# ErlerPhilipp/points2surf

Hardware: NVIDIA H100
Metric: SDF queries/sec at grid_res=256 (higher is better)
Workload: dtype f16 operands / f32 accumulate (wgmma); hi/lo split f16 (fp32-level) for FC tails and guard-band recompute

## Files before the change

### points2surf_b200/csrc/net_tc.cu

```cuda
#include "model.cuh"
#include "tc_ptx.cuh"

namespace p2s {

using namespace ptx;

namespace {

constexpr int kTile = 64;
constexpr int kWG = 2;
constexpr int kThreads = 128 * kWG;
constexpr uint32_t kAct2Bytes = kTile * 128 * 2;
template <bool PRECISE>
struct Cfg {
    static constexpr int kChunks = PRECISE ? 1 : 4;
    static constexpr int kSplit = 8 / kChunks;
    static constexpr uint32_t kChunkBytes = PRECISE ? 65536u : 32768u;
    static constexpr uint32_t kW3Bytes = kChunks * kChunkBytes;
    static constexpr uint32_t kMidScale = PRECISE ? 2u : 1u;
    static constexpr uint32_t kMidBytes = (8192u + 8192u + 16384u) * kMidScale;
    static constexpr uint32_t kPerqBytes = PRECISE ? 16384u : 8192u;
    static constexpr uint32_t kOffMid = kW3Bytes;
    static constexpr uint32_t kWgPerq = kAct2Bytes * kMidScale;
    static constexpr uint32_t kWgWq = kWgPerq + kPerqBytes;
    static constexpr uint32_t kWgBytes = kWgWq + 192 * 4;
    static constexpr uint32_t kOffWg = kOffMid + kMidBytes;
    static constexpr uint32_t kOffBias = kOffWg + kWG * kWgBytes;
    static constexpr uint32_t kSmemBytes = kOffBias + 320 * 4;
};
static_assert(Cfg<false>::kSmemBytes <= 232448 && Cfg<true>::kSmemBytes <= 232448, "shared memory budget");

struct Seg {
    const float* ptr;
    int n;
    int tiles;
    int center;
};

struct PassParams {
    Seg seg[2];
    const float* query;
    const float* R;
    int tiles_per_query;
    int B;
    const float* W0;
    const float* b0;
    int num_mid;
    int mid_N[3];
    const uint8_t* mid_img[3];
    const float* mid_bias[3];
    int perq_layer;
    const uint8_t* perq_img;
    const uint8_t* w3_img;
    float* out;
};

__device__ __forceinline__ uint32_t pack_relu(float a, float b) {
    uint32_t r;
    asm("cvt.rn.relu.satfinite.f16x2.f32 %0, %1, %2;" : "=r"(r) : "f"(b), "f"(a));
    return r;
}
__device__ __forceinline__ void pack_relu_split(float a, float b, uint32_t& hi, uint32_t& lo) {
    hi = pack_relu(a, b);
    const float2 hf = __half22float2(*reinterpret_cast<const __half2*>(&hi));
    lo = pack_half2(fmaxf(a, 0.f) - hf.x, fmaxf(b, 0.f) - hf.y);
}
template <bool PRECISE>
__device__ __forceinline__ void pack_act(float a, float b, uint32_t& hi, uint32_t& lo) {
    if (PRECISE) pack_relu_split(a, b, hi, lo);
    else hi = pack_relu(a, b);
}

template <bool PRECISE, int R>
__device__ __forceinline__ void mid_mma(float (&d)[R], const uint32_t (&a)[4], const uint32_t (&al)[4], uint64_t w, uint64_t w_lo, uint32_t acc) {
    if (R == 32) {
        auto& d32 = reinterpret_cast<float (&)[32]>(d);
        if (PRECISE) { wgmma_rs_n64(d32, al, w, acc); wgmma_rs_n64(d32, a, w_lo, 1); wgmma_rs_n64(d32, a, w, 1); }
        else wgmma_rs_n64(d32, a, w, acc);
    } else {
        auto& d64 = reinterpret_cast<float (&)[64]>(d);
        if (PRECISE) { wgmma_rs_n128(d64, al, w, acc); wgmma_rs_n128(d64, a, w_lo, 1); wgmma_rs_n128(d64, a, w, 1); }
        else wgmma_rs_n128(d64, a, w, acc);
    }
}

template <bool PRECISE>
__global__ void __launch_bounds__(kThreads, 1) pointnet_pass_kernel(const PassParams p) {
    using C = Cfg<PRECISE>;
    constexpr int kL = PRECISE ? 4 : 1;
    extern __shared__ __align__(1024) uint8_t smem[];
    float* s_bias = reinterpret_cast<float*>(smem + C::kOffBias);
    const int tid = threadIdx.x, wg = tid >> 7, t = tid & 127, lane = tid & 31, q4 = lane & 3;
    const int r0 = (t >> 5) * 16 + (lane >> 2);
    const int part = blockIdx.x % C::kSplit;
    const int stream = blockIdx.x / C::kSplit, nstreams = gridDim.x / C::kSplit;
    const int nq = (p.B > stream) ? (p.B - stream + nstreams - 1) / nstreams : 0;
    const int tpq = p.tiles_per_query;
    uint32_t mid_off[3] = {0, 0, 0};
    {
        uint32_t o = 0;
        for (int l = 0; l < p.num_mid; ++l) { mid_off[l] = o; o += (uint32_t)p.mid_N[l] * 128u * C::kMidScale; }
    }

    if (nq > 0) {
        const uint4* src = reinterpret_cast<const uint4*>(p.w3_img + (size_t)part * C::kW3Bytes);
        uint4* dst = reinterpret_cast<uint4*>(smem);
        for (uint32_t i = tid; i < C::kW3Bytes / 16; i += kThreads) dst[i] = src[i];
        for (int l = 0; l < p.num_mid; ++l) {
            if (l == p.perq_layer) continue;
            const uint4* s = reinterpret_cast<const uint4*>(p.mid_img[l]);
            uint4* d = reinterpret_cast<uint4*>(smem + C::kOffMid + mid_off[l]);
            for (uint32_t i = tid; i < (uint32_t)p.mid_N[l] * 8u * C::kMidScale; i += kThreads) d[i] = s[i];
        }
    }
    {
        int off = 0;
        for (int l = 0; l < p.num_mid; ++l) {
            for (int i = tid; i < p.mid_N[l]; i += kThreads) s_bias[off + i] = p.mid_bias[l][i];
            off += p.mid_N[l];
        }
        for (int i = tid; i < 64; i += kThreads) s_bias[256 + i] = p.b0[i];
    }
    fence_proxy_async_smem();
    __syncthreads();

    uint8_t* wsm = smem + C::kOffWg + wg * C::kWgBytes;
    uint8_t* act2 = wsm;
    uint8_t* perq = wsm + C::kWgPerq;
    float* wq = reinterpret_cast<float*>(wsm + C::kWgWq);
    const float* s_b0 = s_bias + 256;
    const uint32_t bar_id = 1 + (uint32_t)wg;
    auto wg_sync = [&]() { asm volatile("bar.sync %0, 128;" ::"r"(bar_id) : "memory"); };
    const uint64_t dsc_act2 = make_smem_desc(smem_u32(act2), 128, 2048);
    const uint64_t dsc_w3 = make_smem_desc(smem_u32(smem), 128, 2048);
    uint64_t dsc_mid[3], dsc_mid_lo[3];
    for (int l = 0; l < 3; ++l) {
        const bool pq = l == p.perq_layer;
        dsc_mid[l] = make_smem_desc(pq ? smem_u32(perq) : smem_u32(smem + C::kOffMid) + mid_off[l], 128, 1024);
        dsc_mid_lo[l] = dsc_mid[l] + (uint64_t)((pq ? 8192u : (uint32_t)p.mid_N[l] * 128u) >> 4);
    }

    for (int qi = wg; qi < nq; qi += kWG) {
        const size_t q = (size_t)stream + (size_t)qi * nstreams;
        wg_sync();
        if (t < 64) {
            const float w0 = p.W0[t * 3 + 0], w1 = p.W0[t * 3 + 1], w2 = p.W0[t * 3 + 2];
            float r[9] = {1.f, 0.f, 0.f, 0.f, 1.f, 0.f, 0.f, 0.f, 1.f};
            if (p.R) {
#pragma unroll
                for (int i = 0; i < 9; ++i) r[i] = p.R[q * 9 + i];
            }
            wq[0 * 64 + t] = w0 * r[0] + w1 * r[3] + w2 * r[6];
            wq[1 * 64 + t] = w0 * r[1] + w1 * r[4] + w2 * r[7];
            wq[2 * 64 + t] = w0 * r[2] + w1 * r[5] + w2 * r[8];
        }
        if (p.perq_layer >= 0) {
            const uint4* s = reinterpret_cast<const uint4*>(p.perq_img + q * C::kPerqBytes);
            uint4* d = reinterpret_cast<uint4*>(perq);
            for (uint32_t i = t; i < C::kPerqBytes / 16; i += 128) d[i] = s[i];
            fence_proxy_async_smem();
        }
        wg_sync();
        float rmax[4 * C::kChunks];
#pragma unroll
        for (int i = 0; i < 4 * C::kChunks; ++i) rmax[i] = -INFINITY;
        for (int tq = 0; tq < tpq; ++tq) {
            const int sgi = tq < p.seg[0].tiles ? 0 : 1;
            const Seg& sg = p.seg[sgi];
            float cx = 0.f, cy = 0.f, cz = 0.f;
            if (sg.center) { cx = p.query[q * 3 + 0]; cy = p.query[q * 3 + 1]; cz = p.query[q * 3 + 2]; }
            float px[2], py[2], pz[2];
#pragma unroll
            for (int h = 0; h < 2; ++h) {
                int local = (tq - (sgi ? p.seg[0].tiles : 0)) * kTile + r0 + 8 * h;
                if (local >= sg.n) local = 0;
                const float* src = sg.ptr + (q * sg.n + local) * 3;
                px[h] = src[0] - cx; py[h] = src[1] - cy; pz[h] = src[2] - cz;
            }
            uint32_t a[4][4], al[4][kL];
#pragma unroll
            for (int kk = 0; kk < 4; ++kk) {
#pragma unroll
                for (int hc = 0; hc < 2; ++hc) {
                    const int ch = kk * 16 + hc * 8 + 2 * q4;
                    const float2 wx = *reinterpret_cast<const float2*>(wq + 0 * 64 + ch);
                    const float2 wy = *reinterpret_cast<const float2*>(wq + 1 * 64 + ch);
                    const float2 wz = *reinterpret_cast<const float2*>(wq + 2 * 64 + ch);
                    const float2 bb = *reinterpret_cast<const float2*>(s_b0 + ch);
#pragma unroll
                    for (int h = 0; h < 2; ++h) {
                        const float v0 = fmaf(wx.x, px[h], fmaf(wy.x, py[h], fmaf(wz.x, pz[h], bb.x)));
                        const float v1 = fmaf(wx.y, px[h], fmaf(wy.y, py[h], fmaf(wz.y, pz[h], bb.y)));
                        pack_act<PRECISE>(v0, v1, a[kk][hc * 2 + h], al[kk][PRECISE ? hc * 2 + h : 0]);
                    }
                }
            }
            int boff = 0;
            for (int l = 0; l < p.num_mid; ++l) {
                const float* bl = s_bias + boff;
                const uint64_t w = dsc_mid[l], w_lo = dsc_mid_lo[l];
                if (l < p.num_mid - 1) {
                    float d[32];
#pragma unroll
                    for (int i = 0; i < 32; ++i) d[i] = 0.f;
                    wgmma_fence();
#pragma unroll
                    for (int ks = 0; ks < 4; ++ks)
                        mid_mma<PRECISE>(d, a[ks], reinterpret_cast<const uint32_t (&)[4]>(al[PRECISE ? ks : 0]), w + (uint64_t)(ks * 16), w_lo + (uint64_t)(ks * 16), ks > 0);
                    wgmma_commit();
                    wgmma_wait<0>();
                    fence_regs(d);
#pragma unroll
                    for (int j = 0; j < 8; ++j) {
                        const float2 bb = *reinterpret_cast<const float2*>(bl + 8 * j + 2 * q4);
                        pack_act<PRECISE>(d[4 * j] + bb.x, d[4 * j + 1] + bb.y, a[j >> 1][(j & 1) * 2], al[j >> 1][PRECISE ? (j & 1) * 2 : 0]);
                        pack_act<PRECISE>(d[4 * j + 2] + bb.x, d[4 * j + 3] + bb.y, a[j >> 1][(j & 1) * 2 + 1], al[j >> 1][PRECISE ? (j & 1) * 2 + 1 : 0]);
                    }
                } else {
                    float d[64];
#pragma unroll
                    for (int i = 0; i < 64; ++i) d[i] = 0.f;
                    wgmma_fence();
#pragma unroll
                    for (int ks = 0; ks < 4; ++ks)
                        mid_mma<PRECISE>(d, a[ks], reinterpret_cast<const uint32_t (&)[4]>(al[PRECISE ? ks : 0]), w + (uint64_t)(ks * 16), w_lo + (uint64_t)(ks * 16), ks > 0);
                    wgmma_commit();
                    wgmma_wait<0>();
                    fence_regs(d);
                    wg_sync();
#pragma unroll
                    for (int j = 0; j < 16; ++j) {
                        const int k = 8 * j + 2 * q4;
                        const float2 bb = *reinterpret_cast<const float2*>(bl + k);
#pragma unroll
                        for (int h = 0; h < 2; ++h) {
                            const int pt = r0 + 8 * h;
                            const uint32_t off = (uint32_t)(pt >> 3) * 2048u + (uint32_t)j * 128u + (uint32_t)(pt & 7) * 16u + (uint32_t)q4 * 4u;
                            uint32_t hi, lo = 0;
                            pack_act<PRECISE>(d[4 * j + 2 * h] + bb.x, d[4 * j + 2 * h + 1] + bb.y, hi, lo);
                            *reinterpret_cast<uint32_t*>(act2 + off) = hi;
                            if (PRECISE) *reinterpret_cast<uint32_t*>(act2 + kAct2Bytes + off) = lo;
                        }
                    }
                    fence_proxy_async_smem();
                    wg_sync();
                }
                boff += p.mid_N[l];
            }
#pragma unroll
            for (int c = 0; c < C::kChunks; ++c) {
                float d0[32], d1[32];
#pragma unroll
                for (int i = 0; i < 32; ++i) { d0[i] = 0.f; d1[i] = 0.f; }
                const uint64_t wa = dsc_w3 + (uint64_t)((uint32_t)c * (C::kChunkBytes >> 4)), wb = wa + (uint64_t)(16384u >> 4);
                wgmma_fence();
#pragma unroll
                for (int ks = 0; ks < 8; ++ks) {
                    const uint64_t x = dsc_act2 + (uint64_t)(ks * 16), o = (uint64_t)(ks * 16);
                    if (PRECISE) {
                        const uint64_t x_lo = x + (uint64_t)(kAct2Bytes >> 4), lo = (uint64_t)(32768u >> 4);
                        wgmma_ss_n64(d0, wa + lo + o, x, ks > 0); wgmma_ss_n64(d0, wa + o, x_lo, 1); wgmma_ss_n64(d0, wa + o, x, 1);
                        wgmma_ss_n64(d1, wb + lo + o, x, ks > 0); wgmma_ss_n64(d1, wb + o, x_lo, 1); wgmma_ss_n64(d1, wb + o, x, 1);
                    } else {
                        wgmma_ss_n64(d0, wa + o, x, ks > 0);
                        wgmma_ss_n64(d1, wb + o, x, ks > 0);
                    }
                }
                wgmma_commit();
                wgmma_wait<0>();
                fence_regs(d0);
                fence_regs(d1);
#pragma unroll
                for (int j = 0; j < 8; ++j) {
                    rmax[4 * c + 0] = fmaxf(rmax[4 * c + 0], fmaxf(d0[4 * j], d0[4 * j + 1]));
                    rmax[4 * c + 1] = fmaxf(rmax[4 * c + 1], fmaxf(d0[4 * j + 2], d0[4 * j + 3]));
                    rmax[4 * c + 2] = fmaxf(rmax[4 * c + 2], fmaxf(d1[4 * j], d1[4 * j + 1]));
                    rmax[4 * c + 3] = fmaxf(rmax[4 * c + 3], fmaxf(d1[4 * j + 2], d1[4 * j + 3]));
                }
            }
        }
#pragma unroll
        for (int i = 0; i < 4 * C::kChunks; ++i) {
            rmax[i] = fmaxf(rmax[i], __shfl_xor_sync(0xffffffffu, rmax[i], 1));
            rmax[i] = fmaxf(rmax[i], __shfl_xor_sync(0xffffffffu, rmax[i], 2));
        }
        if (q4 == 0) {
#pragma unroll
            for (int i = 0; i < 4 * C::kChunks; ++i)
                p.out[q * 1024 + (size_t)((part * C::kChunks + (i >> 2)) * 128 + ((i >> 1) & 1) * 64 + r0 + (i & 1) * 8)] = rmax[i];
        }
    }
}

__global__ void pack_kmajor_kernel(const float* __restrict__ W, int rows, int K, int row0, uint32_t sbo, uint8_t* __restrict__ img, int lo) {
    int e = blockIdx.x * blockDim.x + threadIdx.x;
    if (e >= rows * K) return;
    int r = e / K, k = e % K;
    uint32_t off = (uint32_t)(r >> 3) * sbo + (uint32_t)(k >> 3) * 128u + (uint32_t)(r & 7) * 16u + (uint32_t)(k & 7) * 2u;
    const float w = W[(size_t)(row0 + r) * K + k];
    const __half h = __float2half_rn(w);
    *reinterpret_cast<__half*>(img + off) = lo ? __float2half_rn(w - __half2float(h)) : h;
}

__global__ void pack_perq_kernel(const float* __restrict__ W, int64_t B, uint8_t* __restrict__ img) {
    int64_t e = (int64_t)blockIdx.x * blockDim.x + threadIdx.x;
    if (e >= B * 4096) return;
    int64_t b = e >> 12;
    int r = (int)((e >> 6) & 63), k = (int)(e & 63);
    uint32_t off = (uint32_t)(r >> 3) * 1024u + (uint32_t)(k >> 3) * 128u + (uint32_t)(r & 7) * 16u + (uint32_t)(k & 7) * 2u;
    *reinterpret_cast<__half*>(img + b * 8192 + off) = __float2half_rn(W[e]);
}

__global__ void __launch_bounds__(256) fold_w1_kernel(const float* __restrict__ W1, const float* __restrict__ T, int64_t B, uint8_t* __restrict__ img) {
    __shared__ float sW[64][65];
    __shared__ __align__(16) float sT[64][68];
    const int64_t b = blockIdx.x;
    const int tid = threadIdx.x;
    for (int e = tid; e < 4096; e += 256) {
        const int r = e >> 6, c = e & 63;
        sW[r][c] = W1[e];
        sT[r][c] = T[b * 4096 + e] + (r == c ? 1.0f : 0.0f);
    }
    __syncthreads();
    const int o = tid >> 2, i0 = (tid & 3) * 16;
    float acc[16];
#pragma unroll
    for (int i = 0; i < 16; ++i) acc[i] = 0.f;
    for (int j = 0; j < 64; ++j) {
        const float w = sW[o][j];
#pragma unroll
        for (int i4 = 0; i4 < 4; ++i4) {
            const float4 t4 = *reinterpret_cast<const float4*>(&sT[j][i0 + 4 * i4]);
            acc[4 * i4 + 0] = fmaf(w, t4.x, acc[4 * i4 + 0]);
            acc[4 * i4 + 1] = fmaf(w, t4.y, acc[4 * i4 + 1]);
            acc[4 * i4 + 2] = fmaf(w, t4.z, acc[4 * i4 + 2]);
            acc[4 * i4 + 3] = fmaf(w, t4.w, acc[4 * i4 + 3]);
        }
    }
    uint8_t* dst = img + b * 8192 + (uint32_t)(o >> 3) * 1024u + (uint32_t)(o & 7) * 16u;
#pragma unroll
    for (int h = 0; h < 2; ++h) {
        uint32_t v[4];
#pragma unroll
        for (int e = 0; e < 4; ++e) v[e] = pack_half2(acc[h * 8 + 2 * e], acc[h * 8 + 2 * e + 1]);
        *reinterpret_cast<uint4*>(dst + (uint32_t)(i0 / 8 + h) * 128u) = make_uint4(v[0], v[1], v[2], v[3]);
    }
}

__global__ void fold_fc3_kernel(const float* __restrict__ W1, const float* __restrict__ Wfc3, const float* __restrict__ bfc3,
                                float* __restrict__ G, float* __restrict__ g0) {
    const int oi = blockIdx.x;
    const int o = oi >> 6, i = oi & 63;
    const int k = threadIdx.x;
    float acc = 0.f;
    for (int j = 0; j < 64; ++j) acc = fmaf(W1[o * 64 + j], Wfc3[(size_t)(j * 64 + i) * 256 + k], acc);
    G[(size_t)oi * 256 + k] = acc;
    if (k == 0) {
        float b = W1[o * 64 + i];
        for (int j = 0; j < 64; ++j) b = fmaf(W1[o * 64 + j], bfc3[j * 64 + i], b);
        g0[oi] = b;
    }
}

__global__ void transpose64_kernel(const float* __restrict__ in, float* __restrict__ out, int64_t B) {
    int64_t e = (int64_t)blockIdx.x * blockDim.x + threadIdx.x;
    if (e >= B * 4096) return;
    int64_t b = e >> 12;
    int i = (int)((e >> 6) & 63), j = (int)(e & 63);
    out[e] = in[b * 4096 + j * 64 + i];
}

__global__ void guard_flag_kernel(const float* __restrict__ logits, int od, int64_t B, float band, int32_t* __restrict__ list, int* __restrict__ count, int64_t base, int64_t cap) {
    int64_t i = (int64_t)blockIdx.x * blockDim.x + threadIdx.x;
    if (i >= B) return;
    if (fabsf(logits[i * od + od - 1]) < band) {
        int slot = atomicAdd(count, 1);
        if (slot < cap) list[slot] = (int32_t)(base + i);
    }
}
__global__ void guard_gather_kernel(const float* __restrict__ src, const int32_t* __restrict__ list, int n, int row_floats, float* __restrict__ dst) {
    int64_t e = (int64_t)blockIdx.x * blockDim.x + threadIdx.x;
    if (e >= (int64_t)n * row_floats) return;
    int i = (int)(e / row_floats), j = (int)(e % row_floats);
    dst[e] = src[(int64_t)list[i] * row_floats + j];
}
__global__ void guard_scatter_kernel(const float* __restrict__ src, const int32_t* __restrict__ list, int n, int od, float* __restrict__ logits) {
    int i = blockIdx.x * blockDim.x + threadIdx.x;
    if (i >= n) return;
    for (int j = 0; j < od; ++j) logits[(int64_t)list[i] * od + j] = src[i * od + j];
}
__global__ void guard_scatter_rows_kernel(const float* __restrict__ src, const int32_t* __restrict__ list, int n, int row_floats, float* __restrict__ dst) {
    int64_t e = (int64_t)blockIdx.x * blockDim.x + threadIdx.x;
    if (e >= (int64_t)n * row_floats) return;
    int i = (int)(e / row_floats), j = (int)(e % row_floats);
    dst[(int64_t)list[i] * row_floats + j] = src[e];
}

}

struct TcStack {
    uint8_t* w3_img = nullptr;
    uint8_t* mid_img[3] = {nullptr, nullptr, nullptr};
    uint8_t* w3_img_p = nullptr;
    uint8_t* mid_img_p[3] = {nullptr, nullptr, nullptr};
    const float* mid_bias[3] = {nullptr, nullptr, nullptr};
    int mid_N[3] = {0, 0, 0};
    int num_mid = 0;
    const float* W0 = nullptr;
    const float* b0 = nullptr;
    const float* b3 = nullptr;
};

struct TcFc {
    const Layer* L = nullptr;
    const uint8_t* img = nullptr;
};
struct TcStnFc { TcFc fc1, fc2, fc3; };

struct TcWeights {
    TcStack qstn;
    TcStack stn[2], fin[2];
    TcStnFc qstn_fc, stn_fc[2];
    TcFc head_fc1[2], head_fc2, head_fc3;
    const uint8_t* fold_img[2] = {nullptr, nullptr};
    const float* fold_bias[2] = {nullptr, nullptr};
    bool fc_on_tc = true;
    std::vector<void*> allocs;
    int sm_count = 132;
    bool prof_on = false;
    std::vector<std::pair<cudaEvent_t, cudaEvent_t>> prof_events;
    double prof_flops = 0.0;
    ~TcWeights() {
        for (void* a : allocs) cudaFree(a);
        for (auto& e : prof_events) { cudaEventDestroy(e.first); cudaEventDestroy(e.second); }
    }
};

namespace {

uint8_t* tc_alloc(TcWeights& t, size_t bytes) {
    void* p = nullptr;
    P2S_CUDA(cudaMalloc(&p, bytes));
    P2S_CUDA(cudaMemset(p, 0, bytes));
    t.allocs.push_back(p);
    return (uint8_t*)p;
}

uint8_t* pack_layer(TcWeights& t, const Layer& L, uint32_t sbo, bool split = false) {
    const size_t one = (size_t)L.cout * L.cin * 2;
    uint8_t* img = tc_alloc(t, one * (split ? 2 : 1));
    P2S_LAUNCH(pack_kmajor_kernel, (unsigned)cdiv((int64_t)L.cout * L.cin, 256), 256, 0, 0, L.W, L.cout, L.cin, 0, sbo, img, 0);
    if (split) P2S_LAUNCH(pack_kmajor_kernel, (unsigned)cdiv((int64_t)L.cout * L.cin, 256), 256, 0, 0, L.W, L.cout, L.cin, 0, sbo, img + one, 1);
    return img;
}

uint8_t* pack_w3(TcWeights& t, const Layer& L, bool split = false) {
    P2S_CHECK(L.cout == 1024 && L.cin == 128, "big layer must be 128 -> 1024");
    const size_t chunk = split ? 65536 : 32768;
    uint8_t* img = tc_alloc(t, 8 * chunk);
    for (int c = 0; c < 8; ++c) {
        P2S_LAUNCH(pack_kmajor_kernel, (unsigned)cdiv(128 * 128, 256), 256, 0, 0, L.W, 128, 128, c * 128, 2048u, img + (size_t)c * chunk, 0);
        if (split) P2S_LAUNCH(pack_kmajor_kernel, (unsigned)cdiv(128 * 128, 256), 256, 0, 0, L.W, 128, 128, c * 128, 2048u, img + (size_t)c * chunk + 32768, 1);
    }
    return img;
}

void launch_pass(Model& m, const TcStack& s, const Seg& s0, const Seg& s1, const float* query, const float* R,
                 int64_t B, int perq_layer, const uint8_t* perq_img, float* out, cudaStream_t st, bool precise) {
    PassParams p{};
    p.seg[0] = s0; p.seg[1] = s1;
    p.query = query; p.R = R;
    p.tiles_per_query = s0.tiles + s1.tiles;
    p.B = (int)B;
    p.W0 = s.W0; p.b0 = s.b0;
    p.num_mid = s.num_mid;
    for (int l = 0; l < 3; ++l) { p.mid_N[l] = s.mid_N[l]; p.mid_img[l] = precise ? s.mid_img_p[l] : s.mid_img[l]; p.mid_bias[l] = s.mid_bias[l]; }
    p.perq_layer = perq_layer;
    p.perq_img = perq_img;
    p.w3_img = precise ? s.w3_img_p : s.w3_img;
    p.out = out;
    for (int l = 0; l < s.num_mid; ++l)
        P2S_CHECK(s.mid_N[l] == (l == s.num_mid - 1 ? 128 : 64), "pass kernel: mid layers must be 64 -> 64 ... -> 128");
    TcWeights& t = *m.tc;
    const int split = precise ? Cfg<true>::kSplit : Cfg<false>::kSplit;
    int streams = t.sm_count / split;
    if ((int64_t)streams > B) streams = (int)B;
    const int grid = streams * split;
    cudaEvent_t e0 = nullptr, e1 = nullptr;
    const bool prof = t.prof_on && !precise;
    if (prof) {
        P2S_CUDA(cudaEventCreate(&e0)); P2S_CUDA(cudaEventCreate(&e1));
        P2S_CUDA(cudaEventRecord(e0, st));
    }
    if (precise) P2S_LAUNCH(pointnet_pass_kernel<true>, grid, kThreads, Cfg<true>::kSmemBytes, st, p);
    else P2S_LAUNCH(pointnet_pass_kernel<false>, grid, kThreads, Cfg<false>::kSmemBytes, st, p);
    if (prof) {
        P2S_CUDA(cudaEventRecord(e1, st));
        t.prof_events.emplace_back(e0, e1);
        double mac_pt = 3.0 * 64 + 128.0 * 1024;
        int prev = 64;
        for (int l = 0; l < s.num_mid; ++l) { mac_pt += (double)prev * s.mid_N[l]; prev = s.mid_N[l]; }
        t.prof_flops += 2.0 * mac_pt * (double)(s0.n + s1.n) * (double)B;
    }
}

Seg make_seg(const float* ptr, int n, int center) { return Seg{ptr, n, n > 0 ? (n + kTile - 1) / kTile : 0, center}; }

void run_fc(const TcFc& f, const float* in, int lda, float* out, int ldc, int64_t Bc, bool relu, bool on_tc, cudaStream_t st,
            const float* in_bias = nullptr, bool in_relu = false) {
    const Layer& L = *f.L;
    if (on_tc && f.img) launch_fc_tc(in, lda, f.img, L.b, out, ldc, Bc, L.cout, L.cin, relu, st, 0, in_bias, in_relu);
    else {
        P2S_CHECK(!in_bias, "input bias needs the tensor-core FC kernel");
        launch_gemm_nt(in, 0, lda, L.W, 0, L.b, out, 0, ldc, (int)Bc, L.cout, L.cin, 1, relu, st);
    }
}

void fc_tail(const Layer& b3src, const TcStnFc& s, bool on_tc, const float* gmax_raw, int64_t Bc, float* g, float* f1, float* f2, float* out, cudaStream_t st) {
    if (on_tc && s.fc1.img) run_fc(s.fc1, gmax_raw, 1024, f1, 512, Bc, true, true, st, b3src.b, true);
    else {
        P2S_CUDA(cudaMemcpyAsync(g, gmax_raw, (size_t)Bc * 1024 * 4, cudaMemcpyDeviceToDevice, st));
        launch_bias_act(g, b3src.b, Bc, 1024, true, st);
        run_fc(s.fc1, g, 1024, f1, 512, Bc, true, on_tc, st);
    }
    run_fc(s.fc2, f1, 512, f2, 256, Bc, true, on_tc, st);
    run_fc(s.fc3, f2, 256, out, s.fc3.L->cout, Bc, false, on_tc, st);
}

}

void tc_build(Model& m) {
    P2S_CHECK(m.cfg.net_size == 1024, "tensor-core path needs net_size 1024");
    TcWeights* t = new TcWeights();
    m.tc = t;
    cudaDeviceProp prop;
    P2S_CUDA(cudaGetDeviceProperties(&prop, m.device));
    t->sm_count = prop.multiProcessorCount;
    P2S_CUDA(cudaFuncSetAttribute(pointnet_pass_kernel<false>, cudaFuncAttributeMaxDynamicSharedMemorySize, (int)Cfg<false>::kSmemBytes));
    P2S_CUDA(cudaFuncSetAttribute(pointnet_pass_kernel<true>, cudaFuncAttributeMaxDynamicSharedMemorySize, (int)Cfg<true>::kSmemBytes));
    auto build_stn = [&](TcStack& s, const Stn& stn, const Layer* c0a, const Layer* c0b) {
        if (!c0a) {
            s.W0 = stn.c1.W; s.b0 = stn.c1.b;
            s.num_mid = 1;
            s.mid_img[0] = pack_layer(*t, stn.c2, 1024); s.mid_bias[0] = stn.c2.b; s.mid_N[0] = 128;
            s.mid_img_p[0] = pack_layer(*t, stn.c2, 1024, true);
        } else {
            s.W0 = c0a->W; s.b0 = c0a->b;
            s.num_mid = 3;
            s.mid_img[0] = pack_layer(*t, *c0b, 1024); s.mid_bias[0] = c0b->b; s.mid_N[0] = 64;
            s.mid_img[1] = pack_layer(*t, stn.c1, 1024); s.mid_bias[1] = stn.c1.b; s.mid_N[1] = 64;
            s.mid_img[2] = pack_layer(*t, stn.c2, 1024); s.mid_bias[2] = stn.c2.b; s.mid_N[2] = 128;
            s.mid_img_p[0] = pack_layer(*t, *c0b, 1024, true);
            s.mid_img_p[1] = pack_layer(*t, stn.c1, 1024, true);
            s.mid_img_p[2] = pack_layer(*t, stn.c2, 1024, true);
        }
        s.w3_img_p = pack_w3(*t, stn.c3, true);
        s.w3_img = pack_w3(*t, stn.c3);
        s.b3 = stn.c3.b;
    };
    auto build_fin = [&](TcStack& s, const Feat& f) {
        s.W0 = f.conv0a.W; s.b0 = f.conv0a.b;
        s.num_mid = 3;
        s.mid_img[0] = pack_layer(*t, f.conv0b, 1024); s.mid_bias[0] = f.conv0b.b; s.mid_N[0] = 64;
        s.mid_img[1] = nullptr; s.mid_bias[1] = f.conv1.b; s.mid_N[1] = 64;
        s.mid_img[2] = pack_layer(*t, f.conv2, 1024); s.mid_bias[2] = f.conv2.b; s.mid_N[2] = 128;
        s.mid_img_p[0] = pack_layer(*t, f.conv0b, 1024, true);
        s.mid_img_p[2] = pack_layer(*t, f.conv2, 1024, true);
        s.w3_img_p = pack_w3(*t, f.conv3, true);
        s.w3_img = pack_w3(*t, f.conv3);
        s.b3 = f.conv3.b;
    };
    fc_tc_init();
    t->fc_on_tc = !env_flag("P2S_FC_FP32");
    auto mk_fc = [&](const Layer& L) {
        TcFc f;
        f.L = &L;
        f.img = fc_tc_supported(L.cout, L.cin) ? fc_tc_pack(L, t->allocs) : nullptr;
        return f;
    };
    auto mk_stn_fc = [&](const Stn& s) { TcStnFc r; r.fc1 = mk_fc(s.fc1); r.fc2 = mk_fc(s.fc2); r.fc3 = mk_fc(s.fc3); return r; };
    if (m.shared_qstn) t->qstn_fc = mk_stn_fc(m.point_stn);
    else if (m.global.has_qstn) t->qstn_fc = mk_stn_fc(m.global.stn1);
    t->stn_fc[0] = mk_stn_fc(m.local.stn2);
    t->stn_fc[1] = mk_stn_fc(m.global.stn2);
    for (int br = 0; br < 2; ++br) {
        const Feat& f = br ? m.global : m.local;
        P2S_CHECK(f.stn2.fc3.cout == 4096 && f.stn2.fc3.cin == 256 && f.conv1.cout == 64 && f.conv1.cin == 64, "unexpected STN shape");
        float* G = reinterpret_cast<float*>(tc_alloc(*t, (size_t)4096 * 256 * 4));
        float* g0 = reinterpret_cast<float*>(tc_alloc(*t, 4096 * 4));
        P2S_LAUNCH(fold_fc3_kernel, 4096, 256, 0, 0, f.conv1.W, f.stn2.fc3.W, f.stn2.fc3.b, G, g0);
        t->fold_img[br] = fc_tc_pack_raw(G, 4096, 256, t->allocs);
        t->fold_bias[br] = g0;
    }
    t->head_fc1[0] = mk_fc(m.fc1_local);
    t->head_fc1[1] = mk_fc(m.fc1_global);
    t->head_fc2 = mk_fc(m.fc2);
    t->head_fc3 = mk_fc(m.fc3);
    if (m.shared_qstn) build_stn(t->qstn, m.point_stn, nullptr, nullptr);
    else if (m.global.has_qstn) build_stn(t->qstn, m.global.stn1, nullptr, nullptr);
    build_stn(t->stn[0], m.local.stn2, &m.local.conv0a, &m.local.conv0b);
    build_stn(t->stn[1], m.global.stn2, &m.global.conv0a, &m.global.conv0b);
    build_fin(t->fin[0], m.local);
    build_fin(t->fin[1], m.global);
    P2S_CUDA(cudaDeviceSynchronize());
}

void tc_destroy(Model& m) {
    delete m.tc;
    m.tc = nullptr;
}

void tc_profile_reset(Model& m, bool on) {
    TcWeights& t = *m.tc;
    for (auto& e : t.prof_events) { cudaEventDestroy(e.first); cudaEventDestroy(e.second); }
    t.prof_events.clear();
    t.prof_flops = 0.0;
    t.prof_on = on;
}

void tc_profile_get(Model& m, double* ms, int64_t* launches, double* flops) {
    TcWeights& t = *m.tc;
    double total = 0.0;
    for (auto& e : t.prof_events) {
        P2S_CUDA(cudaEventSynchronize(e.second));
        float x = 0.f;
        P2S_CUDA(cudaEventElapsedTime(&x, e.first, e.second));
        total += x;
    }
    *ms = total;
    *launches = (int64_t)t.prof_events.size();
    *flops = t.prof_flops;
}

static void forward_tc_core(Model& m, const float* patch, const float* sub, const float* query, int64_t B,
                            float* logits, cudaStream_t st, bool precise) {
    TcWeights& t = *m.tc;
    const int P = m.cfg.points_per_patch, S = m.cfg.sub_sample_size;
    const int64_t Bc_max = 8192;
    const size_t per_q = 1024 * 4 + 512 + 256 + 4 + 9 + 4096 * 2 + 1024 + 256 + 128 + 4096  + 16 +
                         1024 + 512 + 256 ;
    float* base = m.ws_net.as<float>(per_q * (size_t)Bc_max + 1024);
    float* pcur = base;
    auto take = [&](size_t n) { float* r = pcur; pcur += (n * (size_t)Bc_max + 63) / 64 * 64; return r; };
    float* gmax = take(1024); float* g = take(1024); float* f1 = take(512); float* f2 = take(256);
    float* q4 = take(4); float* R = take(9); float* T = take(4096); float* Tt = take(4096);
    float* fmax_l = take(1024); float* fmax_g = take(1024); float* cat = take(1024); float* h3 = take(256); float* h4 = take(128);
    uint8_t* perq = reinterpret_cast<uint8_t*>(take(4096));
    uint8_t* imgA = reinterpret_cast<uint8_t*>(take(1024)); uint8_t* imgB = reinterpret_cast<uint8_t*>(take(512)); uint8_t* imgC = reinterpret_cast<uint8_t*>(take(256));
    const bool fc_tc = t.fc_on_tc || precise;
    auto img_ok = [](const TcStnFc& f) { return f.fc1.img && f.fc2.img; };
    auto stn_tail_img = [&](const Layer& c3, const TcStnFc& f, const float* gmax_raw, int64_t Bc, float* out_f2) {
        launch_pack_a(gmax_raw, 1024, Bc, 1024, c3.b, true, imgA, st);
        launch_fc_tc_img(imgA, f.fc1.img, f.fc1.L->b, imgB, 0, Bc, 512, 1024, true, st, 3, 16, 0);
        if (out_f2) launch_fc_tc_img(imgB, f.fc2.img, f.fc2.L->b, out_f2, 256, Bc, 256, 512, true, st, 0);
        else launch_fc_tc_img(imgB, f.fc2.img, f.fc2.L->b, imgC, 0, Bc, 256, 512, true, st, 3, 8, 0);
    };

    for (int64_t b0 = 0; b0 < B; b0 += Bc_max) {
        const int64_t Bc = (B - b0 < Bc_max) ? (B - b0) : Bc_max;
        const float* pa = patch + b0 * P * 3;
        const float* su = sub + b0 * S * 3;
        const float* qu = query + b0 * 3;
        const float* Rq = nullptr;
        if (m.shared_qstn) {
            { StageScope ts("net: pass kernels", st); launch_pass(m, t.qstn, make_seg(pa, P, 0), make_seg(su, S, 1), qu, nullptr, Bc, -1, nullptr, gmax, st, precise); }
            { StageScope ts("net: fc tails", st);
              if (fc_tc && img_ok(t.qstn_fc)) {
                  stn_tail_img(m.point_stn.c3, t.qstn_fc, gmax, Bc, f2);
                  run_fc(t.qstn_fc.fc3, f2, 256, q4, 4, Bc, false, false, st);
              } else fc_tail(m.point_stn.c3, t.qstn_fc, fc_tc, gmax, Bc, g, f1, f2, q4, st); }
            launch_quat_to_rot(q4, R, Bc, st);
            Rq = R;
        } else if (m.global.has_qstn) {
            launch_pass(m, t.qstn, make_seg(su, S, 1), make_seg(nullptr, 0, 0), qu, nullptr, Bc, -1, nullptr, gmax, st, precise);
            if (fc_tc && img_ok(t.qstn_fc)) {
                stn_tail_img(m.global.stn1.c3, t.qstn_fc, gmax, Bc, f2);
                run_fc(t.qstn_fc.fc3, f2, 256, q4, 4, Bc, false, false, st);
            } else fc_tail(m.global.stn1.c3, t.qstn_fc, fc_tc, gmax, Bc, g, f1, f2, q4, st);
            launch_quat_to_rot(q4, R, Bc, st);
            Rq = R;
        }
        for (int br = 1; br >= 0; --br) {
            const Feat& f = br ? m.global : m.local;
            const Seg sg = br ? make_seg(su, S, 1) : make_seg(pa, P, 0);
            float* fmax = br ? fmax_g : fmax_l;
            { StageScope ts("net: pass kernels", st); launch_pass(m, t.stn[br], sg, make_seg(nullptr, 0, 0), qu, Rq, Bc, -1, nullptr, gmax, st, precise); }
            if (fc_tc) {
                StageScope ts("net: fc tails", st);
                if (img_ok(t.stn_fc[br])) {
                    stn_tail_img(f.stn2.c3, t.stn_fc[br], gmax, Bc, nullptr);
                    launch_fc_tc_img(imgC, t.fold_img[br], t.fold_bias[br], perq, 0, Bc, 4096, 256, false, st, precise ? 2 : 1);
                } else {
// ... 86 lines not shown
```

Before: 398,700.

## Pipeline pointnet pass: templated stack, TMA-prefetched per-query weights, overlapped wgmma chunks

Templates the pass kernel on stack depth and per-query layer index so layer offsets are compile-time constants. Per-query weight images are double-buffered and fetched with bulk async copies on mbarriers one query ahead. Point tiles and rotations are prefetched into registers one tile ahead. The 1024-wide conv3 is split into blocks whose wgmma issue overlaps the max-reduction of the previous block and the next tile's early mid layers. This hides global-load and tensor-core latency at the cost of more registers, extra shared memory and more complex synchronisation.

```diff
diff --git a/points2surf_b200/csrc/net_tc.cu b/points2surf_b200/csrc/net_tc.cu
--- a/points2surf_b200/csrc/net_tc.cu
+++ b/points2surf_b200/csrc/net_tc.cu
@@ -20,15 +20,23 @@
     static constexpr uint32_t kMidScale = PRECISE ? 2u : 1u;
     static constexpr uint32_t kMidBytes = (8192u + 8192u + 16384u) * kMidScale;
     static constexpr uint32_t kPerqBytes = PRECISE ? 16384u : 8192u;
+    static constexpr uint32_t kPerqBufs = PRECISE ? 1u : 2u;
     static constexpr uint32_t kOffMid = kW3Bytes;
     static constexpr uint32_t kWgPerq = kAct2Bytes * kMidScale;
-    static constexpr uint32_t kWgWq = kWgPerq + kPerqBytes;
+    static constexpr uint32_t kWgWq = kWgPerq + kPerqBufs * kPerqBytes;
     static constexpr uint32_t kWgBytes = kWgWq + 192 * 4;
     static constexpr uint32_t kOffWg = kOffMid + kMidBytes;
     static constexpr uint32_t kOffBias = kOffWg + kWG * kWgBytes;
-    static constexpr uint32_t kSmemBytes = kOffBias + 320 * 4;
+    static constexpr uint32_t kOffBar = kOffBias + 320 * 4;
+    static constexpr uint32_t kSmemBytes = kOffBar + kWG * 2 * 8;
 };
 static_assert(Cfg<false>::kSmemBytes <= 232448 && Cfg<true>::kSmemBytes <= 232448, "shared memory budget");
+
+template <int NUM_MID>
+struct Stack {
+    static constexpr uint32_t n(int l) { return l == NUM_MID - 1 ? 128u : 64u; }
+    static constexpr uint32_t off(int l) { return l == 0 ? 0u : off(l - 1) + n(l - 1); }
+};
 
 struct Seg {
     const float* ptr;
@@ -45,11 +53,8 @@
     int B;
     const float* W0;
     const float* b0;
-    int num_mid;
-    int mid_N[3];
     const uint8_t* mid_img[3];
     const float* mid_bias[3];
-    int perq_layer;
     const uint8_t* perq_img;
     const uint8_t* w3_img;
     float* out;
@@ -84,10 +89,54 @@
     }
 }
 
-template <bool PRECISE>
+__device__ __forceinline__ void load_tile(const PassParams& p, size_t q, int tq, int r0, float (&x)[2][3], float (&c)[3]) {
+    const bool s1 = tq >= p.seg[0].tiles;
+    const float* ptr = s1 ? p.seg[1].ptr : p.seg[0].ptr;
+    const int n = s1 ? p.seg[1].n : p.seg[0].n;
+    const int tile = s1 ? tq - p.seg[0].tiles : tq;
+#pragma unroll
+    for (int h = 0; h < 2; ++h) {
+        int local = tile * kTile + r0 + 8 * h;
+        if (local >= n) local = 0;
+        const float* src = ptr + (q * n + local) * 3;
+        x[h][0] = src[0]; x[h][1] = src[1]; x[h][2] = src[2];
+    }
+    c[0] = 0.f; c[1] = 0.f; c[2] = 0.f;
+    if (s1 ? p.seg[1].center : p.seg[0].center) { c[0] = p.query[q * 3 + 0]; c[1] = p.query[q * 3 + 1]; c[2] = p.query[q * 3 + 2]; }
+}
+
+template <bool PRECISE, int kL>
+__device__ __forceinline__ void first_layer(const float* wq, const float* s_b0, int q4, const float (&x)[2][3], const float (&c)[3],
+                                            uint32_t (&a)[4][4], uint32_t (&al)[4][kL]) {
+    float px[2], py[2], pz[2];
+#pragma unroll
+    for (int h = 0; h < 2; ++h) { px[h] = x[h][0] - c[0]; py[h] = x[h][1] - c[1]; pz[h] = x[h][2] - c[2]; }
+#pragma unroll
+    for (int kk = 0; kk < 4; ++kk) {
+#pragma unroll
+        for (int hc = 0; hc < 2; ++hc) {
+            const int ch = kk * 16 + hc * 8 + 2 * q4;
+            const float2 wx = *reinterpret_cast<const float2*>(wq + 0 * 64 + ch);
+            const float2 wy = *reinterpret_cast<const float2*>(wq + 1 * 64 + ch);
+            const float2 wz = *reinterpret_cast<const float2*>(wq + 2 * 64 + ch);
+            const float2 bb = *reinterpret_cast<const float2*>(s_b0 + ch);
+#pragma unroll
+            for (int h = 0; h < 2; ++h) {
+                const float v0 = fmaf(wx.x, px[h], fmaf(wy.x, py[h], fmaf(wz.x, pz[h], bb.x)));
+                const float v1 = fmaf(wx.y, px[h], fmaf(wy.y, py[h], fmaf(wz.y, pz[h], bb.y)));
+                pack_act<PRECISE>(v0, v1, a[kk][hc * 2 + h], al[kk][PRECISE ? hc * 2 + h : 0]);
+            }
+        }
+    }
+}
+
+template <bool PRECISE, int NUM_MID, int PERQ_LAYER>
 __global__ void __launch_bounds__(kThreads, 1) pointnet_pass_kernel(const PassParams p) {
     using C = Cfg<PRECISE>;
+    using S = Stack<NUM_MID>;
     constexpr int kL = PRECISE ? 4 : 1;
+    constexpr bool kBulk = PERQ_LAYER >= 0 && !PRECISE;
+    constexpr bool kEarlyMid = !PRECISE && NUM_MID == 3;
     extern __shared__ __align__(1024) uint8_t smem[];
     float* s_bias = reinterpret_cast<float*>(smem + C::kOffBias);
     const int tid = threadIdx.x, wg = tid >> 7, t = tid & 127, lane = tid & 31, q4 = lane & 3;
@@ -96,30 +145,28 @@
     const int stream = blockIdx.x / C::kSplit, nstreams = gridDim.x / C::kSplit;
     const int nq = (p.B > stream) ? (p.B - stream + nstreams - 1) / nstreams : 0;
     const int tpq = p.tiles_per_query;
-    uint32_t mid_off[3] = {0, 0, 0};
-    {
-        uint32_t o = 0;
-        for (int l = 0; l < p.num_mid; ++l) { mid_off[l] = o; o += (uint32_t)p.mid_N[l] * 128u * C::kMidScale; }
-    }
 
     if (nq > 0) {
         const uint4* src = reinterpret_cast<const uint4*>(p.w3_img + (size_t)part * C::kW3Bytes);
         uint4* dst = reinterpret_cast<uint4*>(smem);
         for (uint32_t i = tid; i < C::kW3Bytes / 16; i += kThreads) dst[i] = src[i];
-        for (int l = 0; l < p.num_mid; ++l) {
-            if (l == p.perq_layer) continue;
+#pragma unroll
+        for (int l = 0; l < NUM_MID; ++l) {
+            if (l == PERQ_LAYER) continue;
             const uint4* s = reinterpret_cast<const uint4*>(p.mid_img[l]);
-            uint4* d = reinterpret_cast<uint4*>(smem + C::kOffMid + mid_off[l]);
-            for (uint32_t i = tid; i < (uint32_t)p.mid_N[l] * 8u * C::kMidScale; i += kThreads) d[i] = s[i];
-        }
-    }
-    {
-        int off = 0;
-        for (int l = 0; l < p.num_mid; ++l) {
-            for (int i = tid; i < p.mid_N[l]; i += kThreads) s_bias[off + i] = p.mid_bias[l][i];
-            off += p.mid_N[l];
-        }
-        for (int i = tid; i < 64; i += kThreads) s_bias[256 + i] = p.b0[i];
+            uint4* d = reinterpret_cast<uint4*>(smem + C::kOffMid + S::off(l) * 128u * C::kMidScale);
+            for (uint32_t i = tid; i < S::n(l) * 8u * C::kMidScale; i += kThreads) d[i] = s[i];
+        }
+    }
+#pragma unroll
+    for (int l = 0; l < NUM_MID; ++l)
+        for (int i = tid; i < (int)S::n(l); i += kThreads) s_bias[S::off(l) + i] = p.mid_bias[l][i];
+    for (int i = tid; i < 64; i += kThreads) s_bias[256 + i] = p.b0[i];
+    uint64_t* bar = reinterpret_cast<uint64_t*>(smem + C::kOffBar) + 2 * wg;
+    if (kBulk && t == 0) {
+        mbar_init(&bar[0], 1);
+        mbar_init(&bar[1], 1);
+        fence_mbar_init();
     }
     fence_proxy_async_smem();
     __syncthreads();
@@ -133,151 +180,190 @@
     auto wg_sync = [&]() { asm volatile("bar.sync %0, 128;" ::"r"(bar_id) : "memory"); };
     const uint64_t dsc_act2 = make_smem_desc(smem_u32(act2), 128, 2048);
     const uint64_t dsc_w3 = make_smem_desc(smem_u32(smem), 128, 2048);
-    uint64_t dsc_mid[3], dsc_mid_lo[3];
-    for (int l = 0; l < 3; ++l) {
-        const bool pq = l == p.perq_layer;
-        dsc_mid[l] = make_smem_desc(pq ? smem_u32(perq) : smem_u32(smem + C::kOffMid) + mid_off[l], 128, 1024);
-        dsc_mid_lo[l] = dsc_mid[l] + (uint64_t)((pq ? 8192u : (uint32_t)p.mid_N[l] * 128u) >> 4);
-    }
-
-    for (int qi = wg; qi < nq; qi += kWG) {
-        const size_t q = (size_t)stream + (size_t)qi * nstreams;
+    const uint64_t dsc_mid = make_smem_desc(smem_u32(smem + C::kOffMid), 128, 1024);
+    const uint64_t dsc_perq = make_smem_desc(smem_u32(perq), 128, 1024);
+    auto query_of = [&](int qi) { return (size_t)stream + (size_t)qi * nstreams; };
+    auto copy_perq = [&](int qi, uint32_t buf) {
+        mbar_arrive_expect_tx(&bar[buf], C::kPerqBytes);
+        bulk_g2s(perq + buf * C::kPerqBytes, p.perq_img + query_of(qi) * C::kPerqBytes, C::kPerqBytes, &bar[buf]);
+    };
+
+    float nx[2][3], nc[3];
+    float nr[9] = {1.f, 0.f, 0.f, 0.f, 1.f, 0.f, 0.f, 0.f, 1.f};
+    float w0[3] = {0.f, 0.f, 0.f};
+    auto load_rot = [&](size_t q) {
+        if (t < 64 && p.R) {
+#pragma unroll
+            for (int i = 0; i < 9; ++i) nr[i] = p.R[q * 9 + i];
+        }
+    };
+    if (t < 64) { w0[0] = p.W0[t * 3 + 0]; w0[1] = p.W0[t * 3 + 1]; w0[2] = p.W0[t * 3 + 2]; }
+    if (wg < nq) {
+        load_tile(p, query_of(wg), 0, r0, nx, nc);
+        load_rot(query_of(wg));
+        if (kBulk && t == 0) copy_perq(wg, 0);
+    }
+
+    float d0[32], d1[32];
+#pragma unroll
+    for (int i = 0; i < 32; ++i) { d0[i] = 0.f; d1[i] = 0.f; }
+    uint32_t kq = 0;
+    for (int qi = wg; qi < nq; qi += kWG, ++kq) {
+        const size_t q = query_of(qi);
+        const bool next_q = qi + kWG < nq;
         wg_sync();
+        if (kBulk && t == 0 && next_q) copy_perq(qi + kWG, (kq + 1) & 1);
         if (t < 64) {
-            const float w0 = p.W0[t * 3 + 0], w1 = p.W0[t * 3 + 1], w2 = p.W0[t * 3 + 2];
-            float r[9] = {1.f, 0.f, 0.f, 0.f, 1.f, 0.f, 0.f, 0.f, 1.f};
-            if (p.R) {
-#pragma unroll
-                for (int i = 0; i < 9; ++i) r[i] = p.R[q * 9 + i];
-            }
-            wq[0 * 64 + t] = w0 * r[0] + w1 * r[3] + w2 * r[6];
-            wq[1 * 64 + t] = w0 * r[1] + w1 * r[4] + w2 * r[7];
-            wq[2 * 64 + t] = w0 * r[2] + w1 * r[5] + w2 * r[8];
-        }
-        if (p.perq_layer >= 0) {
+            wq[0 * 64 + t] = w0[0] * nr[0] + w0[1] * nr[3] + w0[2] * nr[6];
+            wq[1 * 64 + t] = w0[0] * nr[1] + w0[1] * nr[4] + w0[2] * nr[7];
+            wq[2 * 64 + t] = w0[0] * nr[2] + w0[1] * nr[5] + w0[2] * nr[8];
+        }
+        if (PERQ_LAYER >= 0 && !kBulk) {
             const uint4* s = reinterpret_cast<const uint4*>(p.perq_img + q * C::kPerqBytes);
             uint4* d = reinterpret_cast<uint4*>(perq);
             for (uint32_t i = t; i < C::kPerqBytes / 16; i += 128) d[i] = s[i];
             fence_proxy_async_smem();
         }
         wg_sync();
+        if (kBulk) mbar_wait_bounded(&bar[kq & 1], (kq >> 1) & 1);
+        const uint64_t dsc_pq = dsc_perq + (uint64_t)(((kq & 1) * C::kPerqBytes * (kBulk ? 1u : 0u)) >> 4);
         float rmax[4 * C::kChunks];
 #pragma unroll
         for (int i = 0; i < 4 * C::kChunks; ++i) rmax[i] = -INFINITY;
+        uint32_t a[4][4], al[4][kL];
+        auto first_and_prefetch = [&](int tq) {
+            first_layer<PRECISE, kL>(wq, s_b0, q4, nx, nc, a, al);
+            if (tq + 1 < tpq) load_tile(p, q, tq + 1, r0, nx, nc);
+            else if (next_q) { load_tile(p, query_of(qi + kWG), 0, r0, nx, nc); load_rot(query_of(qi + kWG)); }
+        };
+        first_and_prefetch(0);
+        auto mid_issue = [&](int l, float (&d)[32]) {
+            const bool pq = l == PERQ_LAYER;
+            const uint64_t w = pq ? dsc_pq : dsc_mid + (uint64_t)((S::off(l) * 128u * C::kMidScale) >> 4);
+            const uint64_t w_lo = w + (uint64_t)((pq ? 8192u : S::n(l) * 128u) >> 4);
+#pragma unroll
+            for (int i = 0; i < 32; ++i) d[i] = 0.f;
+            wgmma_fence();
+#pragma unroll
+            for (int ks = 0; ks < 4; ++ks)
+                mid_mma<PRECISE>(d, a[ks], reinterpret_cast<const uint32_t (&)[4]>(al[PRECISE ? ks : 0]), w + (uint64_t)(ks * 16), w_lo + (uint64_t)(ks * 16), ks > 0);
+            wgmma_commit();
+        };
+        auto mid_finish = [&](int l, float (&d)[32]) {
+            const float* bl = s_bias + S::off(l);
+            fence_regs(d);
+#pragma unroll
+            for (int j = 0; j < 8; ++j) {
+                const float2 bb = *reinterpret_cast<const float2*>(bl + 8 * j + 2 * q4);
+                pack_act<PRECISE>(d[4 * j] + bb.x, d[4 * j + 1] + bb.y, a[j >> 1][(j & 1) * 2], al[j >> 1][PRECISE ? (j & 1) * 2 : 0]);
+                pack_act<PRECISE>(d[4 * j + 2] + bb.x, d[4 * j + 3] + bb.y, a[j >> 1][(j & 1) * 2 + 1], al[j >> 1][PRECISE ? (j & 1) * 2 + 1 : 0]);
+            }
+        };
         for (int tq = 0; tq < tpq; ++tq) {
-            const int sgi = tq < p.seg[0].tiles ? 0 : 1;
-            const Seg& sg = p.seg[sgi];
-            float cx = 0.f, cy = 0.f, cz = 0.f;
-            if (sg.center) { cx = p.query[q * 3 + 0]; cy = p.query[q * 3 + 1]; cz = p.query[q * 3 + 2]; }
-            float px[2], py[2], pz[2];
-#pragma unroll
-            for (int h = 0; h < 2; ++h) {
-                int local = (tq - (sgi ? p.seg[0].tiles : 0)) * kTile + r0 + 8 * h;
-                if (local >= sg.n) local = 0;
-                const float* src = sg.ptr + (q * sg.n + local) * 3;
-                px[h] = src[0] - cx; py[h] = src[1] - cy; pz[h] = src[2] - cz;
+            if (!kEarlyMid || tq == 0) {
+#pragma unroll
+                for (int l = 0; l < NUM_MID - 1; ++l) {
+                    float d[32];
+                    mid_issue(l, d);
+                    wgmma_wait<0>();
+                    mid_finish(l, d);
+                }
             }
-            uint32_t a[4][4], al[4][kL];
-#pragma unroll
-            for (int kk = 0; kk < 4; ++kk) {
-#pragma unroll
-                for (int hc = 0; hc < 2; ++hc) {
-                    const int ch = kk * 16 + hc * 8 + 2 * q4;
-                    const float2 wx = *reinterpret_cast<const float2*>(wq + 0 * 64 + ch);
-                    const float2 wy = *reinterpret_cast<const float2*>(wq + 1 * 64 + ch);
-                    const float2 wz = *reinterpret_cast<const float2*>(wq + 2 * 64 + ch);
-                    const float2 bb = *reinterpret_cast<const float2*>(s_b0 + ch);
+            {
+                constexpr int l = NUM_MID - 1;
+                const float* bl = s_bias + S::off(l);
+                const bool pq = l == PERQ_LAYER;
+                const uint64_t w = pq ? dsc_pq : dsc_mid + (uint64_t)((S::off(l) * 128u * C::kMidScale) >> 4);
+                const uint64_t w_lo = w + (uint64_t)((pq ? 8192u : S::n(l) * 128u) >> 4);
+                float d[64];
+#pragma unroll
+                for (int i = 0; i < 64; ++i) d[i] = 0.f;
+                wgmma_fence();
+#pragma unroll
+                for (int ks = 0; ks < 4; ++ks)
+                    mid_mma<PRECISE>(d, a[ks], reinterpret_cast<const uint32_t (&)[4]>(al[PRECISE ? ks : 0]), w + (uint64_t)(ks * 16), w_lo + (uint64_t)(ks * 16), ks > 0);
+                wgmma_commit();
+                wgmma_wait<0>();
+                fence_regs(d);
+                wg_sync();
+#pragma unroll
+                for (int j = 0; j < 16; ++j) {
+                    const int k = 8 * j + 2 * q4;
+                    const float2 bb = *reinterpret_cast<const float2*>(bl + k);
 #pragma unroll
                     for (int h = 0; h < 2; ++h) {
-                        const float v0 = fmaf(wx.x, px[h], fmaf(wy.x, py[h], fmaf(wz.x, pz[h], bb.x)));
-                        const float v1 = fmaf(wx.y, px[h], fmaf(wy.y, py[h], fmaf(wz.y, pz[h], bb.y)));
-                        pack_act<PRECISE>(v0, v1, a[kk][hc * 2 + h], al[kk][PRECISE ? hc * 2 + h : 0]);
+                        const int pt = r0 + 8 * h;
+                        const uint32_t off = (uint32_t)(pt >> 3) * 2048u + (uint32_t)j * 128u + (uint32_t)(pt & 7) * 16u + (uint32_t)q4 * 4u;
+                        uint32_t hi, lo = 0;
+                        pack_act<PRECISE>(d[4 * j + 2 * h] + bb.x, d[4 * j + 2 * h + 1] + bb.y, hi, lo);
+                        *reinterpret_cast<uint32_t*>(act2 + off) = hi;
+                        if (PRECISE) *reinterpret_cast<uint32_t*>(act2 + kAct2Bytes + off) = lo;
                     }
                 }
+                fence_proxy_async_smem();
+                wg_sync();
             }
-            int boff = 0;
-            for (int l = 0; l < p.num_mid; ++l) {
-                const float* bl = s_bias + boff;
-                const uint64_t w = dsc_mid[l], w_lo = dsc_mid_lo[l];
-                if (l < p.num_mid - 1) {
-                    float d[32];
-#pragma unroll
-                    for (int i = 0; i < 32; ++i) d[i] = 0.f;
-                    wgmma_fence();
-#pragma unroll
-                    for (int ks = 0; ks < 4; ++ks)
-                        mid_mma<PRECISE>(d, a[ks], reinterpret_cast<const uint32_t (&)[4]>(al[PRECISE ? ks : 0]), w + (uint64_t)(ks * 16), w_lo + (uint64_t)(ks * 16), ks > 0);
-                    wgmma_commit();
-                    wgmma_wait<0>();
-                    fence_regs(d);
-#pragma unroll
-                    for (int j = 0; j < 8; ++j) {
-                        const float2 bb = *reinterpret_cast<const float2*>(bl + 8 * j + 2 * q4);
-                        pack_act<PRECISE>(d[4 * j] + bb.x, d[4 * j + 1] + bb.y, a[j >> 1][(j & 1) * 2], al[j >> 1][PRECISE ? (j & 1) * 2 : 0]);
-                        pack_act<PRECISE>(d[4 * j + 2] + bb.x, d[4 * j + 3] + bb.y, a[j >> 1][(j & 1) * 2 + 1], al[j >> 1][PRECISE ? (j & 1) * 2 + 1 : 0]);
-                    }
-                } else {
-                    float d[64];
-#pragma unroll
-                    for (int i = 0; i < 64; ++i) d[i] = 0.f;
-                    wgmma_fence();
-#pragma unroll
-                    for (int ks = 0; ks < 4; ++ks)
-                        mid_mma<PRECISE>(d, a[ks], reinterpret_cast<const uint32_t (&)[4]>(al[PRECISE ? ks : 0]), w + (uint64_t)(ks * 16), w_lo + (uint64_t)(ks * 16), ks > 0);
-                    wgmma_commit();
-                    wgmma_wait<0>();
-                    fence_regs(d);
-                    wg_sync();
-#pragma unroll
-                    for (int j = 0; j < 16; ++j) {
-                        const int k = 8 * j + 2 * q4;
-                        const float2 bb = *reinterpret_cast<const float2*>(bl + k);
-#pragma unroll
-                        for (int h = 0; h < 2; ++h) {
-                            const int pt = r0 + 8 * h;
-                            const uint32_t off = (uint32_t)(pt >> 3) * 2048u + (uint32_t)j * 128u + (uint32_t)(pt & 7) * 16u + (uint32_t)q4 * 4u;
-                            uint32_t hi, lo = 0;
-                            pack_act<PRECISE>(d[4 * j + 2 * h] + bb.x, d[4 * j + 2 * h + 1] + bb.y, hi, lo);
-                            *reinterpret_cast<uint32_t*>(act2 + off) = hi;
-                            if (PRECISE) *reinterpret_cast<uint32_t*>(act2 + kAct2Bytes + off) = lo;
-                        }
-                    }
-                    fence_proxy_async_smem();
-                    wg_sync();
-                }
-                boff += p.mid_N[l];
-            }
-#pragma unroll
-            for (int c = 0; c < C::kChunks; ++c) {
-                float d0[32], d1[32];
-#pragma unroll
-                for (int i = 0; i < 32; ++i) { d0[i] = 0.f; d1[i] = 0.f; }
-                const uint64_t wa = dsc_w3 + (uint64_t)((uint32_t)c * (C::kChunkBytes >> 4)), wb = wa + (uint64_t)(16384u >> 4);
+            auto issue = [&](int b, float (&d)[32]) {
+                const uint64_t wa = dsc_w3 + (uint64_t)((uint32_t)(b >> 1) * (C::kChunkBytes >> 4) + (uint32_t)(b & 1) * (16384u >> 4));
                 wgmma_fence();
 #pragma unroll
                 for (int ks = 0; ks < 8; ++ks) {
                     const uint64_t x = dsc_act2 + (uint64_t)(ks * 16), o = (uint64_t)(ks * 16);
                     if (PRECISE) {
                         const uint64_t x_lo = x + (uint64_t)(kAct2Bytes >> 4), lo = (uint64_t)(32768u >> 4);
-                        wgmma_ss_n64(d0, wa + lo + o, x, ks > 0); wgmma_ss_n64(d0, wa + o, x_lo, 1); wgmma_ss_n64(d0, wa + o, x, 1);
-                        wgmma_ss_n64(d1, wb + lo + o, x, ks > 0); wgmma_ss_n64(d1, wb + o, x_lo, 1); wgmma_ss_n64(d1, wb + o, x, 1);
+                        wgmma_ss_n64(d, wa + lo + o, x, ks > 0); wgmma_ss_n64(d, wa + o, x_lo, 1); wgmma_ss_n64(d, wa + o, x, 1);
                     } else {
-                        wgmma_ss_n64(d0, wa + o, x, ks > 0);
-                        wgmma_ss_n64(d1, wb + o, x, ks > 0);
+                        wgmma_ss_n64(d, wa + o, x, ks > 0);
                     }
                 }
                 wgmma_commit();
-                wgmma_wait<0>();
-                fence_regs(d0);
-                fence_regs(d1);
+            };
+            auto reduce = [&](int b, float (&d)[32]) {
+                fence_regs(d);
 #pragma unroll
                 for (int j = 0; j < 8; ++j) {
-                    rmax[4 * c + 0] = fmaxf(rmax[4 * c + 0], fmaxf(d0[4 * j], d0[4 * j + 1]));
-                    rmax[4 * c + 1] = fmaxf(rmax[4 * c + 1], fmaxf(d0[4 * j + 2], d0[4 * j + 3]));
-                    rmax[4 * c + 2] = fmaxf(rmax[4 * c + 2], fmaxf(d1[4 * j], d1[4 * j + 1]));
-                    rmax[4 * c + 3] = fmaxf(rmax[4 * c + 3], fmaxf(d1[4 * j + 2], d1[4 * j + 3]));
+                    rmax[2 * b + 0] = fmaxf(rmax[2 * b + 0], fmaxf(d[4 * j], d[4 * j + 1]));
+                    rmax[2 * b + 1] = fmaxf(rmax[2 * b + 1], fmaxf(d[4 * j + 2], d[4 * j + 3]));
                 }
+            };
+            constexpr int kBlocks = 2 * C::kChunks;
+            const bool more = tq + 1 < tpq;
+            if (kEarlyMid && more) {
+                first_and_prefetch(tq + 1);
+                issue(0, d0);
+                mid_issue(0, d1);
+                wgmma_wait<1>();
+                reduce(0, d0);
+                issue(1, d0);
+                wgmma_wait<1>();
+                mid_finish(0, d1);
+                mid_issue(1, d1);
+                wgmma_wait<1>();
+                reduce(1, d0);
+                issue(2, d0);
+                wgmma_wait<1>();
+                mid_finish(1, d1);
+                issue(3, d1);
+                wgmma_wait<1>();
+                reduce(2, d0);
+#pragma unroll
+                for (int b = 4; b < kBlocks; ++b) {
+                    issue(b, (b & 1) ? d1 : d0);
+                    wgmma_wait<1>();
+                    reduce(b - 1, (b & 1) ? d0 : d1);
+                }
+            } else {
+                issue(0, d0);
+#pragma unroll
+                for (int b = 1; b < kBlocks; ++b) {
+                    issue(b, (b & 1) ? d1 : d0);
+                    wgmma_wait<1>();
+                    reduce(b - 1, (b & 1) ? d0 : d1);
+                }
+                if (more) first_and_prefetch(tq + 1);
             }
+            wgmma_wait<0>();
+            reduce(kBlocks - 1, d1);
         }
 #pragma unroll
         for (int i = 0; i < 4 * C::kChunks; ++i) {
@@ -473,14 +559,18 @@
     p.tiles_per_query = s0.tiles + s1.tiles;
     p.B = (int)B;
     p.W0 = s.W0; p.b0 = s.b0;
-    p.num_mid = s.num_mid;
-    for (int l = 0; l < 3; ++l) { p.mid_N[l] = s.mid_N[l]; p.mid_img[l] = precise ? s.mid_img_p[l] : s.mid_img[l]; p.mid_bias[l] = s.mid_bias[l]; }
-    p.perq_layer = perq_layer;
+    for (int l = 0; l < 3; ++l) { p.mid_img[l] = precise ? s.mid_img_p[l] : s.mid_img[l]; p.mid_bias[l] = s.mid_bias[l]; }
     p.perq_img = perq_img;
     p.w3_img = precise ? s.w3_img_p : s.w3_img;
     p.out = out;
     for (int l = 0; l < s.num_mid; ++l)
         P2S_CHECK(s.mid_N[l] == (l == s.num_mid - 1 ? 128 : 64), "pass kernel: mid layers must be 64 -> 64 ... -> 128");
+    P2S_CHECK((s.num_mid == 1 && perq_layer < 0) || (s.num_mid == 3 && (perq_layer < 0 || perq_layer == 1)),
+              "pass kernel: stack must be 1 mid layer, or 3 with the per-query layer (if any) second");
+    P2S_CHECK(p.tiles_per_query > 0, "pass kernel: empty point set");
+    void (*kern)(const PassParams);
+    if (precise) kern = s.num_mid == 1 ? pointnet_pass_kernel<true, 1, -1> : perq_layer < 0 ? pointnet_pass_kernel<true, 3, -1> : pointnet_pass_kernel<true, 3, 1>;
+    else kern = s.num_mid == 1 ? pointnet_pass_kernel<false, 1, -1> : perq_layer < 0 ? pointnet_pass_kernel<false, 3, -1> : pointnet_pass_kernel<false, 3, 1>;
     TcWeights& t = *m.tc;
     const int split = precise ? Cfg<true>::kSplit : Cfg<false>::kSplit;
     int streams = t.sm_count / split;
@@ -492,8 +582,7 @@
         P2S_CUDA(cudaEventCreate(&e0)); P2S_CUDA(cudaEventCreate(&e1));
         P2S_CUDA(cudaEventRecord(e0, st));
     }
-    if (precise) P2S_LAUNCH(pointnet_pass_kernel<true>, grid, kThreads, Cfg<true>::kSmemBytes, st, p);
-    else P2S_LAUNCH(pointnet_pass_kernel<false>, grid, kThreads, Cfg<false>::kSmemBytes, st, p);
+    P2S_LAUNCH(kern, grid, kThreads, precise ? Cfg<true>::kSmemBytes : Cfg<false>::kSmemBytes, st, p);
     if (prof) {
         P2S_CUDA(cudaEventRecord(e1, st));
         t.prof_events.emplace_back(e0, e1);
@@ -536,8 +625,10 @@
     cudaDeviceProp prop;
     P2S_CUDA(cudaGetDeviceProperties(&prop, m.device));
     t->sm_count = prop.multiProcessorCount;
-    P2S_CUDA(cudaFuncSetAttribute(pointnet_pass_kernel<false>, cudaFuncAttributeMaxDynamicSharedMemorySize, (int)Cfg<false>::kSmemBytes));
-    P2S_CUDA(cudaFuncSetAttribute(pointnet_pass_kernel<true>, cudaFuncAttributeMaxDynamicSharedMemorySize, (int)Cfg<true>::kSmemBytes));
+    for (auto kern : {pointnet_pass_kernel<false, 1, -1>, pointnet_pass_kernel<false, 3, -1>, pointnet_pass_kernel<false, 3, 1>})
+        P2S_CUDA(cudaFuncSetAttribute(kern, cudaFuncAttributeMaxDynamicSharedMemorySize, (int)Cfg<false>::kSmemBytes));
+    for (auto kern : {pointnet_pass_kernel<true, 1, -1>, pointnet_pass_kernel<true, 3, -1>, pointnet_pass_kernel<true, 3, 1>})
+        P2S_CUDA(cudaFuncSetAttribute(kern, cudaFuncAttributeMaxDynamicSharedMemorySize, (int)Cfg<true>::kSmemBytes));
     auto build_stn = [&](TcStack& s, const Stn& stn, const Layer* c0a, const Layer* c0b) {
         if (!c0a) {
             s.W0 = stn.c1.W; s.b0 = stn.c1.b;
```

Result: faster. 426,400 (median of 6 runs) (+7.0%).
